# SysSec-KAIST/LTESniffer

Measured on AMD Instinct MI355X. Metric: subframes/s (20 MHz, 150 RNTIs), higher is better.
Workload: dtype f32+int16

## Files before the change

include/ltesniffer_amd.h:

```cpp
#ifndef LTESNIFFER_AMD_H
#define LTESNIFFER_AMD_H
#include <stddef.h>
#include <stdint.h>
#ifdef __cplusplus
extern "C" {
#endif

#define LSN_SUCCESS 0
#define LSN_ERROR (-1)
#define LSN_ERROR_INVALID_INPUTS (-2)
#define LSN_ERROR_NO_DEVICE (-3)

typedef struct lsn_phy lsn_phy_t;
typedef struct lsn_worker lsn_worker_t;

typedef struct {
  uint32_t nof_prb;
  uint32_t nof_ports;
  uint32_t id;
  uint32_t cp;
  uint32_t phich_length;
  uint32_t phich_resources;
  uint32_t frame_type;
} lsn_cell_t;
// ... 198 lines not shown
  float offset_freq_hz;
  uint32_t start_tti;
  uint32_t update_meta_period;
  uint64_t max_subframes;
  uint64_t subframes_done;
  int status;
} lsn_file_cell_t;
int lsn_file_process_cells(const char* path, const lsn_file_cfg_t* cfg , double sample_rate_hz,
                           lsn_file_cell_t* cells, uint32_t n_cells);
typedef struct {
  int64_t in_lo, in_hi;
  uint32_t blk_used, nof_active;
  uint64_t first_subframe[LSN_FILE_MAX_CELLS];
  uint32_t nof_subframes[LSN_FILE_MAX_CELLS];
  uint32_t taps[LSN_FILE_MAX_CELLS];
} lsn_file_cells_span_t;
int lsn_file_cells_span(const lsn_file_cfg_t* cfg, double sample_rate_hz, const lsn_file_cell_t* cells, uint32_t n_cells, uint64_t in_end ,
                        uint32_t block, uint32_t blk_subframes, lsn_file_cells_span_t* out);
int lsn_resample_cells(int device, const void* in, int in_on_device, uint64_t n_in, const lsn_resample_cfg_t* cfgs, uint32_t n_cells, float* const* outs,
                       int out_on_device, const uint64_t* n_out);

int lsn_resample_cells_ring(int device, const void* in, uint64_t n_in, uint64_t ring_samples, const lsn_resample_cfg_t* cfgs, uint32_t n_cells, float* const* outs,
                            const uint64_t* n_out);

typedef struct lsn_stream lsn_stream_t;
typedef struct {
  uint32_t struct_size;
  int      device;
  double   sample_rate_hz;
  uint32_t nof_antennas;
  uint32_t sample_format;
  float    sample_scale;
  uint32_t block_subframes;
  uint64_t ring_samples;
} lsn_stream_cfg_t;
typedef struct {
  uint64_t samples_pushed;
  uint64_t ring_samples;
  int64_t  oldest_needed;
  uint32_t block_subframes, nof_cells;
  int      failed;
  int      status[LSN_FILE_MAX_CELLS];
  uint64_t subframes_submitted[LSN_FILE_MAX_CELLS];
} lsn_stream_status_t;
typedef struct {
  uint64_t ring_samples, block_input;
// ... 282 lines not shown
```

ltesniffer_amd/__init__.py:

```python
import ctypes as C
import os
import struct
import subprocess

import numpy as np


_HERE = os.path.dirname(os.path.abspath(__file__))
LIB_PATH = os.environ.get("LSN_LIB_PATH") or os.path.join(_HERE, "lib", "libltesniffer_amd.so")

LSN_SUCCESS, LSN_ERROR, LSN_ERROR_INVALID_INPUTS, LSN_ERROR_NO_DEVICE = 0, -1, -2, -3
TAP_GRID, TAP_CE, TAP_PDCCH_LLR, TAP_CHEST, TAP_CFI, TAP_CANDIDATES, TAP_CCE_POWER, TAP_ACCEPTED, TAP_RB_POWER = range(9)
TAP_PDSCH_JOBS, TAP_PDSCH_LLR16, TAP_RM_WORDS, TAP_CB_RESULT = 9, 10, 11, 12
KERNELS = ["k_ofdm", "k_chest", "k_chest_fin", "k_pcfich", "k_pdcch_llr", "k_cce_power", "k_viterbi", "k_pdsch_prep",
           "k_pdsch_demod", "k_turbo<64>", "k_rb_power", "k_turbo<128>", "k_rm"]

EXPORTS = ["lsn_phy_create", "lsn_phy_destroy", "lsn_phy_set_cell", "lsn_phy_get_avail", "lsn_phy_put_pending",
           "lsn_phy_join_pending", "lsn_phy_set_pdu_sink", "lsn_phy_get_stats", "lsn_phy_get_est_cfo",
           "lsn_phy_add_evergreen", "lsn_phy_add_forbidden", "lsn_phy_setup_default_rnti_intervals",
           "lsn_phy_nof_active_rnti", "lsn_phy_get_ue_config", "lsn_worker_buffers", "lsn_worker_buffer_len", "lsn_worker_prepare",
           "lsn_worker_sf_idx", "lsn_worker_sfn", "lsn_phy_process_device", "lsn_phy_process_host", "lsn_phy_process_host_int", "lsn_phy_tap",
           "lsn_phy_get_perf", "lsn_kernel_name", "lsn_version", "lsn_pcap_open", "lsn_pcap_open_mem",
           "lsn_pcap_set_wall_clock", "lsn_pcap_write", "lsn_pcap_sink", "lsn_pcap_mem", "lsn_pcap_nof_records",
           "lsn_pcap_reset", "lsn_pcap_close", "lsn_phy_set_pcap_writer", "lsn_phy_set_api_mode", "lsn_phy_tracked_ul_modulation", "lsn_phy_set_ul_config", "lsn_phy_get_ul_config", "lsn_sib2_decode", "lsn_phy_pusch_decode",
           "lsn_phy_tap_ul", "lsn_phy_set_prach_config", "lsn_phy_prach_detect", "lsn_phy_set_prach_sink", "lsn_prach_tti_opportunity", "lsn_phy_process_file", "lsn_phy_mib_decode", "lsn_phy_mib_decode_llr", "lsn_phy_submit_device", "lsn_phy_wait", "lsn_cell_search",
           "lsn_phy_set_shortcut_discovery", "lsn_phy_get_shortcut_discovery", "lsn_phy_set_histogram_threshold", "lsn_phy_print_stats",
           "lsn_phy_set_mcs_update_interval", "lsn_phy_update_mcs_database", "lsn_phy_nof_tracked_rnti", "lsn_worker_buffers_offset", "lsn_pcap_digest", "lsn_pcap_set_store", "lsn_pcap_set_digest_blocks", "lsn_pcap_block_digests", "lsn_phy_create_multi", "lsn_phy_nof_devices",
           "lsn_phy_set_cfo_correction", "lsn_phy_get_cfo_correction", "lsn_phy_set_candidate_pruning", "lsn_phy_set_stage_c_taps", "lsn_phy_prepare_file", "lsn_phy_get_meta_formats", "lsn_phy_nof_workers", "lsn_phy_worker",
           "lsn_phy_set_sampling", "lsn_phy_get_sampling", "lsn_symbol_sz", "lsn_sampling_freq_hz", "lsn_cell_search_rates",
           "lsn_resample", "lsn_resample_span", "lsn_phy_process_file_rate", "lsn_resample_cells", "lsn_file_cells_span", "lsn_file_process_cells",
           "lsn_clock_plan", "lsn_clock_fit", "lsn_clock_replica", "lsn_clock_track", "lsn_clock_estimate", "lsn_file_clock_estimate",
           "lsn_carrier_scan_plan", "lsn_carrier_scan_decide", "lsn_carrier_scan", "lsn_file_carrier_scan", "lsn_carrier_channel", "lsn_carrier_channel_span",
           "lsn_phy_set_channel_filter", "lsn_channel_filter_design", "lsn_channel_filter", "lsn_channel_filter_span", "lsn_cells_stopbands",
           "lsn_resample_cells_ring", "lsn_stream_open", "lsn_stream_push", "lsn_stream_flush", "lsn_stream_status", "lsn_stream_close", "lsn_stream_span",
           "lsn_stream_track", "lsn_stream_track_status", "lsn_stream_track_step", "lsn_pss_timing", "lsn_pss_timing_error"]

RATES_3GPP, RATES_SRSRAN = 0, 1


def symbol_sz(nof_prb, rates=RATES_3GPP):
    return int(lib().lsn_symbol_sz(int(nof_prb), int(rates)))


def sampling_freq_hz(nof_prb, rates=RATES_3GPP):
    return int(lib().lsn_sampling_freq_hz(int(nof_prb), int(rates)))


def turbo_nwin(K):
    p1 = p2 = 1
    for P in range(min(K // 32, 128), 0, -1):
        if K % P == 0:
            p2 = P
            break
    for P in range(min(K // 32, 64), 0, -1):
        if K % P == 0:
            p1 = P
            break
    return p2 if p2 >= 96 else p1
# ... 342 lines not shown
        L.lsn_phy_set_pcap_writer.argtypes = [C.c_void_p, C.c_void_p]
        L.lsn_phy_set_ul_config.argtypes = [C.c_void_p, C.POINTER(UlCfg)]
        L.lsn_phy_tracked_ul_modulation.argtypes = [C.c_void_p, C.c_uint16]
        L.lsn_phy_set_api_mode.argtypes = [C.c_void_p, C.c_int, API_SINK, C.c_void_p, C.c_void_p]
        L.lsn_phy_get_ul_config.argtypes = [C.c_void_p, C.POINTER(UlCfg), C.POINTER(Sib2), C.POINTER(C.c_uint32)]
        L.lsn_sib2_decode.argtypes = [C.c_char_p, C.c_uint32, C.POINTER(Sib2)]
        L.lsn_phy_pusch_decode.argtypes = [C.c_void_p, C.c_void_p, C.c_int, C.c_uint32, C.c_uint32, C.c_void_p, C.c_uint32, C.c_void_p,
                                           C.c_void_p, C.c_size_t]
        L.lsn_phy_tap_ul.argtypes = [C.c_void_p, C.c_int, C.c_uint32, C.c_void_p, C.c_size_t]
        L.lsn_phy_tap_ul.restype = C.c_long
        L.lsn_phy_submit_device.argtypes = [C.c_void_p, C.c_void_p, C.c_uint32, C.c_uint32, C.c_uint32, C.c_void_p]
        L.lsn_phy_wait.argtypes = [C.c_void_p]
        L.lsn_phy_mib_decode.argtypes = [C.c_void_p, C.c_void_p, C.c_int, C.POINTER(Mib)]
        L.lsn_phy_mib_decode_llr.argtypes = [C.c_void_p, C.c_void_p, C.c_int, C.POINTER(Mib), C.c_void_p]
        L.lsn_phy_process_file.argtypes = [C.c_void_p, C.c_char_p, C.POINTER(FileCfg), C.c_uint32, C.c_uint64, C.c_uint32, C.POINTER(C.c_uint64)]
        L.lsn_phy_prepare_file.argtypes = [C.c_void_p, C.c_uint32]
        L.lsn_phy_process_file_rate.argtypes = [C.c_void_p, C.c_char_p, C.POINTER(FileCfg), C.POINTER(FileRate), C.c_uint32, C.c_uint64, C.c_uint32, C.POINTER(C.c_uint64)]
        L.lsn_resample.argtypes = [C.c_int, C.c_void_p, C.c_int, C.c_uint64, C.POINTER(ResampleCfg), C.c_void_p, C.c_int, C.c_uint64]
        L.lsn_resample_span.argtypes = [C.POINTER(ResampleCfg), C.c_uint64, C.c_uint64, C.POINTER(ResampleSpan)]
        L.lsn_resample_cells.argtypes = [C.c_int, C.c_void_p, C.c_int, C.c_uint64, C.POINTER(ResampleCfg), C.c_uint32, C.POINTER(C.c_void_p), C.c_int, C.POINTER(C.c_uint64)]
        L.lsn_file_cells_span.argtypes = [C.POINTER(FileCfg), C.c_double, C.POINTER(FileCell), C.c_uint32, C.c_uint64, C.c_uint32, C.c_uint32, C.POINTER(FileCellsSpan)]
        L.lsn_file_process_cells.argtypes = [C.c_char_p, C.POINTER(FileCfg), C.c_double, C.POINTER(FileCell), C.c_uint32]
        L.lsn_resample_cells_ring.argtypes = [C.c_int, C.c_void_p, C.c_uint64, C.c_uint64, C.POINTER(ResampleCfg), C.c_uint32, C.POINTER(C.c_void_p), C.POINTER(C.c_uint64)]
        L.lsn_stream_open.argtypes = [C.POINTER(StreamCfg), C.POINTER(FileCell), C.c_uint32, C.POINTER(C.c_void_p)]
        L.lsn_stream_push.argtypes = [C.c_void_p, C.c_void_p, C.c_uint64]
        L.lsn_stream_flush.argtypes = [C.c_void_p]
        L.lsn_stream_status.argtypes = [C.c_void_p, C.POINTER(StreamStatus)]
        L.lsn_stream_close.argtypes = [C.c_void_p]
        L.lsn_stream_span.argtypes = [C.POINTER(StreamCfg), C.POINTER(FileCell), C.c_uint32, C.c_uint64, C.POINTER(StreamSpan)]
        L.lsn_stream_track.argtypes = [C.c_void_p, C.POINTER(StreamTrackCfg)]
        L.lsn_stream_track_status.argtypes = [C.c_void_p, C.POINTER(StreamTrackStatus)]
        L.lsn_stream_track_step.argtypes = [C.POINTER(StreamTrackCfg), C.c_double, C.c_double, C.c_uint32, C.POINTER(StreamTrackState), C.c_double, C.c_int,
                                            C.POINTER(C.c_uint64), C.POINTER(C.c_uint64)]
        L.lsn_pss_timing.argtypes = [C.c_int, C.c_int, C.POINTER(PssTimingCell), C.c_uint32]
        L.lsn_pss_timing_error.argtypes = [C.c_void_p, C.c_uint32, C.POINTER(C.c_double), C.POINTER(C.c_double)]
        L.lsn_phy_set_prach_config.argtypes = [C.c_void_p, C.POINTER(PrachCfg)]
        L.lsn_phy_prach_detect.argtypes = [C.c_void_p, C.c_void_p, C.c_int, C.c_uint32, C.c_uint32, C.POINTER(PrachDet), C.c_uint32]
        L.lsn_phy_set_prach_sink.argtypes = [C.c_void_p, PRACH_SINK, C.c_void_p]
        L.lsn_phy_set_prach_sink.restype = None
        L.lsn_prach_tti_opportunity.argtypes = [C.c_uint32, C.c_uint32]
        L.lsn_phy_set_shortcut_discovery.argtypes = [C.c_void_p, C.c_int]
        L.lsn_phy_get_shortcut_discovery.argtypes = [C.c_void_p]
        L.lsn_phy_set_histogram_threshold.argtypes = [C.c_void_p, C.c_uint32]
        L.lsn_phy_print_stats.argtypes = [C.c_void_p, C.c_void_p]
        L.lsn_phy_set_mcs_update_interval.argtypes = [C.c_void_p, C.c_uint32]
        L.lsn_phy_update_mcs_database.argtypes = [C.c_void_p]
# ... 546 lines not shown
    n_in, nant = iq.shape[0], iq.shape[1]
    n = len(cells)
    cfgs = (ResampleCfg * max(n, 1))()
    counts = (C.c_uint64 * max(n, 1))()
    outs = []
    for i, c in enumerate(cells):
        cfgs[i] = _resample_cfg(nant, rate_in, c["rate_out"], c.get("first_sample", 0), c.get("first_frac", 0.0), in_base, c.get("out_first", 0), c.get("passband_hz", 0.0),
                                sample_format, sample_scale, c.get("center_offset_hz", 0.0))
        k = c.get("n_out", n_out)
        if k is None:
            sp = ResampleSpan()
            _check(lib().lsn_resample_span(C.byref(cfgs[i]), 0, int(in_base) + n_in, C.byref(sp)), "lsn_resample_span")
            k = int(sp.max_out)
        counts[i] = int(k)
        outs.append(np.zeros((nant, int(k)), dtype=np.complex64))
    ptrs = (C.c_void_p * max(n, 1))(*[o.ctypes.data for o in outs])
    rc = lib().lsn_resample_cells_ring(device, iq.ctypes.data, n_in, int(ring_samples), cfgs, n, ptrs, counts)
    if rc == LSN_ERROR_INVALID_INPUTS:
        raise ValueError("resample_cells_ring: refused")
    _check(rc, "lsn_resample_cells_ring")
    return outs


def channel_filter_design(rate_in, passband_hz, stopband_hz):
    import numpy as np
    d = ChannelFilterDesign(C.sizeof(ChannelFilterDesign), 0, 0, 0, 0.0)
    taps = np.zeros(2 * 512 + 1, dtype=np.float32)
    rc = lib().lsn_channel_filter_design(float(rate_in), float(passband_hz), float(stopband_hz), C.byref(d), taps.ctypes.data, taps.size)
    if rc == LSN_ERROR_INVALID_INPUTS:
        raise ValueError("channel filter: refused")
    _check(rc, "lsn_channel_filter_design")
    return dict(L=int(d.half_len), fc=float(d.cutoff), taps=taps[:d.nof_taps].copy())


def _channel_filter_cfg(nof_antennas, rate_in, passband_hz, stopband_hz, center_offset_hz, in_base, out_first, sample_format, sample_scale):
    return ChannelFilterCfg(C.sizeof(ChannelFilterCfg), int(nof_antennas), int(sample_format), float(sample_scale), float(rate_in), float(passband_hz), float(stopband_hz),
                            float(center_offset_hz), int(in_base), int(out_first))


def channel_filter_span(n_out, in_end, rate_in, passband_hz, stopband_hz, out_first=0, center_offset_hz=0.0):
    cfg = _channel_filter_cfg(1, rate_in, passband_hz, stopband_hz, center_offset_hz, 0, out_first, FILE_CF32, 0.0)
    sp = ResampleSpan()
    rc = lib().lsn_channel_filter_span(C.byref(cfg), int(n_out), int(in_end), C.byref(sp))
    if rc == LSN_ERROR_INVALID_INPUTS:
        raise ValueError("channel filter: refused")
    _check(rc, "lsn_channel_filter_span")
# ... 392 lines not shown
```

ltesniffer_amd/csrc/host/lsn_capi.cc:

```cpp
#include "lsn_engine.h"
#include "lsn_cells.h"
#include "lsn_chanfilt_launch.h"
#include "lsn_stream_ring.h"
#include <chrono>
#include <condition_variable>
#include <deque>
#include <mutex>
#include <thread>
#include <time.h>

struct lsn_worker {
  lsn_phy* phy = nullptr;
  float* buf[LSN_MAX_RX] = {nullptr, nullptr};
  float* buf_offset[2] = {nullptr, nullptr};
  uint32_t buf_len = 0;
  uint32_t index = 0;
  uint32_t sf_idx = 0, sfn = 0;
  int update_meta = 0;
  lsn_dl_sf_cfg_t sf_cfg{};
};

struct lsn_phy {
  std::unique_ptr<lsn::Engine> engine;
  std::vector<std::unique_ptr<lsn::Engine>> more;
// ... 767 lines not shown
      raw = d_in;
    }
    cf32* dst = (cf32*)out;
    const size_t out_bytes = (size_t)n_out * nant * sizeof(cf32);
    if (!out_on_device) {
      HIP_CHECK(hipMalloc(&d_out, out_bytes));
      dst = (cf32*)d_out;
    }
    LsnChanFirCell k;
    k.taps = d_taps; k.L = f.L; k.w = f.tune; k.nco = d_nco; k.out = dst; k.out_first = (int64_t)cfg->out_first; k.n_out = n_out;
    lsn_launch_chan_fir(raw, fmt, sfm.scale, need_lo, len, nant, &k, 1, st);
    if (!out_on_device) HIP_CHECK(hipMemcpyAsync(out, d_out, out_bytes, hipMemcpyDeviceToHost, st));
    HIP_CHECK(hipStreamSynchronize(st));
  } catch (const std::exception& ex) {
    fprintf(stderr, "ltesniffer_amd: channel_filter: %s\n", ex.what());
    rc = LSN_ERROR;
  }
  if (st) (void)hipStreamDestroy(st);
  if (d_in) (void)hipFree(d_in);
  if (d_taps) (void)hipFree(d_taps);
  if (d_out) (void)hipFree(d_out);
  return rc;
}
int lsn_phy_prepare_file(lsn_phy_t* phy, uint32_t nof_antennas)
{
  if (!phy) return LSN_ERROR_INVALID_INPUTS;
  return phy->engine->reserveFileBuffers(nof_antennas);
}
int lsn_phy_set_ul_config(lsn_phy_t* phy, const lsn_ul_cfg_t* cfg)
{
  if (!phy || !cfg) return LSN_ERROR_INVALID_INPUTS;
  return phy->engine->setUlConfig(*cfg);
}
static void sib2_to_c(const lsn::Sib2Config& c, lsn_sib2_t* o)
{
  o->n_sb = c.n_sb; o->hopping_mode = c.hopping_mode; o->pusch_hop_offset = c.pusch_hop_offset; o->enable_64qam = c.enable_64qam;
  o->group_hopping_enabled = c.group_hopping_enabled; o->group_assignment_pusch = c.group_assignment_pusch;
  o->sequence_hopping_enabled = c.sequence_hopping_enabled; o->cyclic_shift = c.cyclic_shift;
  o->root_seq_idx = c.root_seq_idx; o->prach_config_idx = c.prach_config_idx; o->high_speed_flag = c.high_speed_flag;
  o->zero_corr_zone = c.zero_corr_zone; o->prach_freq_offset = c.prach_freq_offset;
}
int lsn_phy_get_ul_config(lsn_phy_t* phy, lsn_ul_cfg_t* ul, lsn_sib2_t* sib2, uint32_t* from_sib2)
{
  if (!phy) return LSN_ERROR_INVALID_INPUTS;
  lsn::Sib2Config s;
  if (!phy->engine->getUlConfig(ul, nullptr, &s)) return 0;
// ... 105 lines not shown
```

ltesniffer_amd/csrc/kernels/lsn_rm.h:

```cpp
#pragma once
#include <stdint.h>
#ifndef LSN_HD
#ifdef __HIPCC__
#define LSN_HD __host__ __device__ __forceinline__
#else
#define LSN_HD static inline
#endif
#endif

struct LsnRmGeom {
  int K, D, R, KP, ND, F, Ncb, nn, nn0, k0, cum_k0;
  int pre01[33];
  int pre2[33];
  uint8_t cnt01[32];
  uint8_t first2[32];
};

LSN_HD int lsn_perm_tc_f(int c) { return ((c & 1) << 4) | ((c & 2) << 2) | (c & 4) | ((c & 8) >> 2) | ((c & 16) >> 4); }

LSN_HD int lsn_rm_nb01_cr(const LsnRmGeom& g, int col, int row)
{
  if (col >= 32) return g.pre01[32];
  const int c = g.cnt01[col];
  return g.pre01[col] + (row < c ? row : c);
// ... 79 lines not shown
LSN_HD int lsn_rm_col_of(int y)
{
#ifdef __HIP_DEVICE_COMPILE__
  return (int)(__builtin_bitreverse32((uint32_t)y) >> 27);
#else
  return lsn_perm_tc_f(y & 31);
#endif
}
LSN_HD void lsn_rm_rank01_fast(LsnRmCol e, int nn, int y, int* r0, int* r1)
{
  const int row = y >> 5, cnt = e.a & 255, m = row < cnt ? row : cnt;
  int a = (e.a >> 8) + row - m;
  int b = (e.b >> 8) + 2 * row - m - (row > 0 ? (e.b & 1) : 0);
  *r0 = a < 0 ? a + nn : a;
  *r1 = b < 0 ? b + nn : b;
}
LSN_HD int lsn_rm_rank2_fast(LsnRmCol e, int nn, int z)
{
  const int row = z >> 5, cnt = e.a & 255, m = row < cnt ? row : cnt;
  const int b = (e.b >> 8) + 2 * row - m - (row > 0 ? (e.b & 1) : 0) + (row < cnt ? 0 : 1);
  return b < 0 ? b + nn : b;
}

LSN_HD int lsn_turbo_nwin(int K)
{
  int p1 = 1, p2 = 1;
  for (int P = (K / 32 < 128 ? K / 32 : 128); P >= 1; P--)
    if (K % P == 0) { p2 = P; break; }
  for (int P = (K / 32 < 64 ? K / 32 : 64); P >= 1; P--)
    if (K % P == 0) { p1 = P; break; }
  return p2 >= 96 ? p2 : p1;
}
#define LSN_TURBO_ONE_WAVE_KMAX 3072
LSN_HD int lsn_turbo_il_words(int K) { const int P = lsn_turbo_nwin(K), W = K / P; return ((W + 1) / 2) * P; }
LSN_HD bool lsn_turbo_two_wave_class(int K) { return lsn_turbo_nwin(K) > 64 || K > LSN_TURBO_ONE_WAVE_KMAX; }
```

ltesniffer_amd/csrc/kernels/lsn_rows.h:

```cpp
#pragma once
#include <stdint.h>
#ifndef LSN_HD
#ifdef __HIPCC__
#define LSN_HD __host__ __device__ __forceinline__
#else
#define LSN_HD static inline
#endif
#endif

#define LSN_ROWS_PER_ITEM 16u
#define LSN_ROWS_DIV_SHIFT 20

struct LsnRowGeom {
  uint32_t n[2];
  uint32_t div_m[2];
  uint32_t rows0;
  uint32_t rows;
};

LSN_HD uint32_t lsn_rows_ordinal(const uint32_t mask[4], uint32_t prb)
{
  uint32_t n = 0;
  for (uint32_t w = 0; w < 4; w++) {
    const uint32_t lo = 32u * w;
// ... 10 lines not shown
    g.n[s] = lsn_rows_ordinal(prb_mask[s], nof_prb);
    g.div_m[s] = g.n[s] ? (1u << LSN_ROWS_DIV_SHIFT) / g.n[s] + 1u : 0u;
  }
  g.rows0 = (nslot - l0) * g.n[0];
  g.rows = g.rows0 + nslot * g.n[1];
  return g;
}

LSN_HD uint32_t lsn_rows_items(const LsnRowGeom& g) { return (g.rows + LSN_ROWS_PER_ITEM - 1u) / LSN_ROWS_PER_ITEM; }

LSN_HD void lsn_rows_locate(const LsnRowGeom& g, uint32_t l0, uint32_t nslot, uint32_t row, uint32_t* l, uint32_t* slot, uint32_t* ord)
{
  const uint32_t s = row >= g.rows0 ? 1u : 0u;
  const uint32_t r = s ? row - g.rows0 : row, n = s ? g.n[1] : g.n[0], m = s ? g.div_m[1] : g.div_m[0];
  const uint32_t q = (r * m) >> LSN_ROWS_DIV_SHIFT;
  *slot = s;
  *l = (s ? nslot : l0) + q;
  *ord = r - q * n;
}

LSN_HD uint32_t lsn_rows_sym_off(uint32_t nof_prb) { return 14u * nof_prb; }
LSN_HD uint32_t lsn_rows_list_off(uint32_t nof_prb) { return 14u * nof_prb + 16u; }
LSN_HD uint32_t lsn_rows_prefix_len(uint32_t nof_prb) { return 15u * nof_prb + 16u; }
```

ltesniffer_amd/csrc/kernels/stage_c.hip:

```cpp
#include "lsn_dsp.h"
#include <algorithm>
#include "lsn_rm.h"
#include <type_traits>

#define SQRT1_2F 0.70710678118654752440f
#define SQRT2F 1.41421356237309504880f
#define LLR_Q 180.0f

__global__ __launch_bounds__(64) void k_pdsch_prep_up(LsnCellDev c, const LsnGrantDev* __restrict__ jobs_h, LsnGrantDev* __restrict__ jobs_d, uint32_t njobs,
                                                      LsnCopySegs sg, uint16_t* __restrict__ prefix)
{
  const int lane = threadIdx.x, nprb = (int)c.nof_prb;
  if (blockIdx.x >= njobs) {
    const uint32_t w = blockIdx.x - njobs, nw = gridDim.x - njobs;
    for (uint32_t q = 0; q < sg.n; q++) {
      const uint32_t words = sg.words[q];
      const bool al = ((((uintptr_t)sg.src[q]) | ((uintptr_t)sg.dst[q])) & 15u) == 0;
      const uint32_t n16 = al ? words / 4 : 0;
      const uint4* a4 = (const uint4*)sg.src[q];
      uint4* b4 = (uint4*)sg.dst[q];
      for (uint32_t i = w * 64u + (uint32_t)lane; i < n16; i += nw * 64u) b4[i] = a4[i];
      const uint32_t* a = (const uint32_t*)sg.src[q];
      uint32_t* b = (uint32_t*)sg.dst[q];
      for (uint32_t i = n16 * 4 + w * 64u + (uint32_t)lane; i < words; i += nw * 64u) b[i] = a[i];
    }
    return;
  }
  __shared__ LsnGrantDev gs;
  constexpr int NW = (int)(sizeof(LsnGrantDev) / 4);
  static_assert(NW <= 64 && sizeof(LsnGrantDev) % 4 == 0, "one word per lane");
  if (lane < NW) {
    const uint32_t v = ((const uint32_t*)(jobs_h + blockIdx.x))[lane];
    ((uint32_t*)&gs)[lane] = v;
    ((uint32_t*)(jobs_d + blockIdx.x))[lane] = v;
  }
  __syncthreads();
  const LsnGrantDev& g = gs;
  uint16_t* pf = prefix + g.prefix_off;
  const int cls = g.sf_idx == 0 ? 0 : (g.sf_idx == 5 ? 1 : 2);
  uint32_t before = 0;
  for (int l = 0; l < 14; l++) {
    uint32_t run = 0;
    for (int base = 0; base < nprb; base += 64) {
      const int prb = base + lane;
      uint32_t v = 0;
      if (prb < nprb && l >= (int)g.l0 && ((g.prb_mask[l >= (int)c.nslot ? 1 : 0][prb >> 5] >> (prb & 31)) & 1u)) v = (uint32_t)__popc((unsigned)c.validmask[(cls * 14 + l) * nprb + prb]);
      uint32_t inc = v;
#pragma unroll
      for (int off = 1; off < 64; off <<= 1) {
        const uint32_t t = __shfl_up(inc, off);
        if (lane >= off) inc += t;
      }
      if (prb < nprb) pf[l * nprb + prb] = (uint16_t)(run + inc - v);
      run += __shfl(inc, 63);
    }
    if (lane == 0) pf[lsn_rows_sym_off((uint32_t)nprb) + l] = (uint16_t)before;
    before += run;
  }
  if (lane == 0) pf[lsn_rows_sym_off((uint32_t)nprb) + 14] = (uint16_t)before;
  uint8_t* pl = (uint8_t*)(pf + lsn_rows_list_off((uint32_t)nprb));
  for (int s = 0; s < 2; s++)
    for (int prb = lane; prb < nprb; prb += 64)
      if ((g.prb_mask[s][prb >> 5] >> (prb & 31)) & 1u) pl[s * nprb + (int)lsn_rows_ordinal(g.prb_mask[s], (uint32_t)prb)] = (uint8_t)prb;
}
void lsn_launch_pdsch_prep_up(const LsnCellDev& c, const LsnGrantDev* jobs_host, LsnGrantDev* jobs_dev, uint32_t njobs, const LsnCopySegs& sg, uint16_t* prefix, hipStream_t s)
{
  uint32_t total = 0;
  for (uint32_t q = 0; q < sg.n; q++) total += sg.words[q];
  const uint32_t ncopy = total ? std::max<uint32_t>(1u, std::min<uint32_t>((total / 4 + 63u) / 64u, 256u)) : 0u;
  LSN_LAUNCH(k_pdsch_prep_up, dim3(njobs + ncopy), dim3(64), 0, s, c, jobs_host, jobs_dev, njobs, sg, prefix);
}

__device__ __forceinline__ int lsn_cvt_sat(float r)
{
  int q;
  asm("v_cvt_i32_f32 %0, %1" : "=v"(q) : "v"(r));
  return q;
}
template <int QM>
__device__ __forceinline__ void emit_q(const LsnCellDev& c, cf32 x, float w, float inv_amp, uint32_t cinit, uint32_t idx, int16_t* __restrict__ out)
{
  float L[8];
  const float wq = w * LLR_Q;
  lsn_demod_llr(QM, x.r * inv_amp, x.i * inv_amp, L);
  const uint32_t n0 = idx * (uint32_t)QM;
  uint32_t x1w[2] = {0u, 0u}, m[8];
// ... 168 lines not shown
        float det = a * d - (br * br + bi * bi);
        cf32 x0, x1;
        x0.r = (d * z0r - (br * z1r - bi * z1i)) / det;
        x0.i = (d * z0i - (br * z1i + bi * z1r)) / det;
        x1.r = (a * z1r - (br * z0r + bi * z0i)) / det;
        x1.i = (a * z1i - (br * z0i - bi * z0r)) / det;
        float w0 = det / d * 4.0f / chan_ref, w1 = det / a * 4.0f / chan_ref;
        if (g.qm[0]) emit(c, (int)g.qm[0], x0, w0, inv_amp, g.cinit[0], idx, out0);
        if (g.qm[1]) emit(c, (int)g.qm[1], x1, w1, inv_amp, g.cinit[1], idx, out1);
      }
      break;
    }
  }
#undef GRID
#undef CE
}
void lsn_launch_pdsch_demod(const LsnCellDev& c, const LsnGrantDev* g, const uint32_t* items, uint32_t nitems, const uint16_t* prefix, const cf32* grid,
                            const cf32* ce, const LsnChest* ch, int16_t* llr, hipStream_t s)
{
  if (nitems) LSN_LAUNCH(k_pdsch_demod, dim3(nitems), dim3(192), 0, s, c, g, items, prefix, grid, ce, ch, llr);
}

#define RM_NT 256
template <bool STAGED>
__device__ __forceinline__ int rm_sum(const int16_t* __restrict__ e, const int16_t* es, int rank, int E, int nn)
{
  int acc = 0;
  for (int k = rank; k < E; k += nn) acc += STAGED ? (int)es[k] : (int)e[k];
  return acc > LSN_LLR_CLIP ? LSN_LLR_CLIP : (acc < -LSN_LLR_CLIP ? -LSN_LLR_CLIP : acc);
}
__global__ __launch_bounds__(RM_NT) void k_rm(const LsnCbDev* __restrict__ cbs, const int16_t* __restrict__ llr, uint32_t* __restrict__ spp_g, uint32_t seg)
{
  extern __shared__ __attribute__((aligned(16))) unsigned char rm_smem[];
  __shared__ LsnRmGeom geom;
  __shared__ LsnRmCol tab[32];
  int16_t* es = (int16_t*)rm_smem;
  const LsnCbDev cb = cbs[blockIdx.x];
  const int tid = threadIdx.x, K = (int)cb.K, F = (int)cb.F, E = (int)cb.E;
  const int P = cb.nwin ? (int)cb.nwin : lsn_turbo_nwin(K), W = K / P;
  const int ND = 32 * ((K + 4 + 31) >> 5) - (K + 4);
  const int16_t* e = llr + cb.e_off;
  const bool staged = (uint32_t)E <= seg;
  if (tid < 64) {
    int c01 = 0, f2 = 0, c2 = 0;
    if (tid < 32) lsn_rm_geom_col(ND, F, tid, &c01, &f2, &c2);
    int i01 = c01, i2 = c2;
#pragma unroll
    for (int off = 1; off < 32; off <<= 1) {
      const int t = __shfl_up(i01, off), u = __shfl_up(i2, off);
      if (tid >= off) { i01 += t; i2 += u; }
    }
    if (tid < 32) { geom.cnt01[tid] = (uint8_t)c01; geom.first2[tid] = (uint8_t)f2; geom.pre01[tid] = i01 - c01; geom.pre2[tid] = i2 - c2; }
    if (tid == 31) { geom.pre01[32] = i01; geom.pre2[32] = i2; }
    __builtin_amdgcn_fence(__ATOMIC_RELEASE, "wavefront"); __builtin_amdgcn_wave_barrier(); __builtin_amdgcn_fence(__ATOMIC_ACQUIRE, "wavefront");
    if (tid == 0) lsn_rm_geom_finish(geom, K, F, (int)cb.rv);
    __builtin_amdgcn_fence(__ATOMIC_RELEASE, "wavefront"); __builtin_amdgcn_wave_barrier(); __builtin_amdgcn_fence(__ATOMIC_ACQUIRE, "wavefront");
    if (tid < 32) tab[tid] = lsn_rm_fast_col(geom, tid);
  }
  if (staged) {
    const uintptr_t a0 = (uintptr_t)e & ~(uintptr_t)15;
    const int skew = (int)(((uintptr_t)e - a0) >> 1);
    const uint4* src = (const uint4*)a0;
    const int end = skew + E, vend = end >> 3;
    for (int v = tid; v <= vend; v += RM_NT) {
      uint4 d = make_uint4(0u, 0u, 0u, 0u);
      if (8 * v < end) d = src[v];
      if (v == vend) {
        const int q = end & 7;
        const uint32_t keep = (q & 1) ? 0x0000FFFFu : 0u;
        switch (q >> 1) { case 0: d.x &= keep; break; case 1: d.y &= keep; break; case 2: d.z &= keep; break; default: d.w &= keep; break; }
      }
      ((uint4*)es)[v] = d;
    }
    es += skew;
  }
  __syncthreads();
  const int nn = geom.nn;
  uint32_t* out = spp_g + cb.spp_off;
  const bool single = staged && E <= nn;
  auto streams = [&](int x, int& v0, int& v1, int& v2) {
    const int y = x + ND;
    int r0, r1;
    lsn_rm_rank01_fast(tab[lsn_rm_col_of(y)], nn, y, &r0, &r1);
    const int r2 = lsn_rm_rank2_fast(tab[lsn_rm_col_of(y - 1)], nn, y - 1);
    if (single) {
      v0 = (int)es[r0 < E ? r0 : E]; v1 = (int)es[r1 < E ? r1 : E]; v2 = (int)es[r2 < E ? r2 : E];
    } else if (staged) {
      v0 = rm_sum<true>(e, es, r0, E, nn); v1 = rm_sum<true>(e, es, r1, E, nn); v2 = rm_sum<true>(e, es, r2, E, nn);
    } else {
      v0 = rm_sum<false>(e, es, r0, E, nn); v1 = rm_sum<false>(e, es, r1, E, nn); v2 = rm_sum<false>(e, es, r2, E, nn);
    }
  };
  int tq = tid / P, tr = tid - tq * P;
  const int dq = RM_NT / P, dr = RM_NT - dq * P;
  for (int t = tid; t < K; t += RM_NT, tq += dq, tr += dr) {
    if (tr >= P) { tr -= P; tq++; }
    const int x = (int)__umul24((uint32_t)tr, (uint32_t)W) + tq;
    int v0, v1, v2;
    streams(x, v0, v1, v2);
    if (x < F) v0 = v1 = -LSN_LLR_CLIP;
    out[t] = ((uint32_t)v0 & 0x3FFu) | (((uint32_t)v1 & 0x3FFu) << 10) | (((uint32_t)v2 & 0x3FFu) << 20);
  }
  if (tid < 4) {
    int v0, v1, v2;
    streams(K + tid, v0, v1, v2);
    out[K + tid] = (uint32_t)v0; out[K + 4 + tid] = (uint32_t)v1; out[K + 8 + tid] = (uint32_t)v2;
  }
}
void lsn_launch_rm(const LsnCbDev* cb, const int16_t* llr, uint32_t* spp, uint32_t ncb, uint32_t emax, hipStream_t s)
{
  static std::atomic<uint64_t> attr_done{0};
  lsn_func_max_lds((const void*)k_rm, 65536, attr_done, "k_rm");
  const uint32_t cap = (65536 - 32) / 2;
  const uint32_t seg = emax < cap ? emax : cap;
  const size_t lds = (((size_t)seg + 16) * 2 + 15) & ~(size_t)15;
  if (ncb) LSN_LAUNCH(k_rm, dim3(ncb), dim3(RM_NT), lds, s, cb, llr, spp, seg);
}

__global__ __launch_bounds__(256) void k_harq_combine(const LsnCbDev* __restrict__ cbs, const uint32_t* __restrict__ keep, uint32_t* pool, uint32_t* scratch, uint32_t copy)
{
  const LsnCbDev cb = cbs[blockIdx.x];
  const uint32_t place = cb.reserved >> 30, off = cb.reserved & 0x3FFFFFFFu;
  const uint32_t* a = (place == 0u ? (const uint32_t*)pool : place == 1u ? (const uint32_t*)scratch : keep) + off;
  const int K = (int)cb.K;
  if (copy) {
    uint32_t* d = pool + cb.spp_off;
    for (int t = threadIdx.x; t < K + 12; t += 256) d[t] = a[t];
    return;
  }
// ... 231 lines not shown
```

Before: 285,400.

## Precompute rate-match walk tables and fuse PDSCH prefix scan with DPP

Rewrites the rate-dematching kernel so each thread derives its LLR byte offsets from per-column walk bases precomputed in LDS. This replaces per-element rank arithmetic, using med3 clamping and direct LDS address-space loads, and specialises the kernel on mode and filler presence. The PDSCH prefix kernel packs two symbols and the PRB-list ordinal into one word and scans them with DPP, which removes the separate PRB list pass and the shuffle-based scan. It also adds a standalone lsn_rm_blocks test entry point. The risk is correctness around the packed bit fields and the filler/head handling.

Result: no change. 289,300, median of 6 (+1.4%).

```diff
diff --git a/include/ltesniffer_amd.h b/include/ltesniffer_amd.h
--- a/include/ltesniffer_amd.h
+++ b/include/ltesniffer_amd.h
@@ -244,6 +244,11 @@
 
 int lsn_resample_cells_ring(int device, const void* in, uint64_t n_in, uint64_t ring_samples, const lsn_resample_cfg_t* cfgs, uint32_t n_cells, float* const* outs,
                             const uint64_t* n_out);
+
+typedef struct {
+  uint32_t K, F, E, rv, nwin, e_off, spp_off;
+} lsn_rm_block_t;
+int lsn_rm_blocks(int device, uint32_t n, const lsn_rm_block_t* blocks, const int16_t* e, uint64_t n_e, uint32_t* words, uint64_t n_words);
 
 typedef struct lsn_stream lsn_stream_t;
 typedef struct {
diff --git a/ltesniffer_amd/__init__.py b/ltesniffer_amd/__init__.py
--- a/ltesniffer_amd/__init__.py
+++ b/ltesniffer_amd/__init__.py
@@ -33,7 +33,7 @@
            "lsn_carrier_scan_plan", "lsn_carrier_scan_decide", "lsn_carrier_scan", "lsn_file_carrier_scan", "lsn_carrier_channel", "lsn_carrier_channel_span",
            "lsn_phy_set_channel_filter", "lsn_channel_filter_design", "lsn_channel_filter", "lsn_channel_filter_span", "lsn_cells_stopbands",
            "lsn_resample_cells_ring", "lsn_stream_open", "lsn_stream_push", "lsn_stream_flush", "lsn_stream_status", "lsn_stream_close", "lsn_stream_span",
-           "lsn_stream_track", "lsn_stream_track_status", "lsn_stream_track_step", "lsn_pss_timing", "lsn_pss_timing_error"]
+           "lsn_stream_track", "lsn_stream_track_status", "lsn_stream_track_step", "lsn_pss_timing", "lsn_pss_timing_error", "lsn_rm_blocks"]
 
 RATES_3GPP, RATES_SRSRAN = 0, 1
 
@@ -422,6 +422,7 @@
         L.lsn_file_cells_span.argtypes = [C.POINTER(FileCfg), C.c_double, C.POINTER(FileCell), C.c_uint32, C.c_uint64, C.c_uint32, C.c_uint32, C.POINTER(FileCellsSpan)]
         L.lsn_file_process_cells.argtypes = [C.c_char_p, C.POINTER(FileCfg), C.c_double, C.POINTER(FileCell), C.c_uint32]
         L.lsn_resample_cells_ring.argtypes = [C.c_int, C.c_void_p, C.c_uint64, C.c_uint64, C.POINTER(ResampleCfg), C.c_uint32, C.POINTER(C.c_void_p), C.POINTER(C.c_uint64)]
+        L.lsn_rm_blocks.argtypes = [C.c_int, C.c_uint32, C.POINTER(RmBlock), C.c_void_p, C.c_uint64, C.c_void_p, C.c_uint64]
         L.lsn_stream_open.argtypes = [C.POINTER(StreamCfg), C.POINTER(FileCell), C.c_uint32, C.POINTER(C.c_void_p)]
         L.lsn_stream_push.argtypes = [C.c_void_p, C.c_void_p, C.c_uint64]
         L.lsn_stream_flush.argtypes = [C.c_void_p]
@@ -1014,6 +1015,24 @@
     return outs
 
 
+class RmBlock(C.Structure):
+    _fields_ = [(n, C.c_uint32) for n in ("K", "F", "E", "rv", "nwin", "e_off", "spp_off")]
+
+
+def rm_blocks(blocks, e, n_words, device=0):
+    import numpy as np
+    e = np.ascontiguousarray(e, dtype=np.int16)
+    arr = (RmBlock * max(len(blocks), 1))()
+    for i, b in enumerate(blocks):
+        arr[i] = RmBlock(int(b["K"]), int(b["F"]), int(b["E"]), int(b["rv"]), int(b.get("nwin", 0)), int(b["e_off"]), int(b["spp_off"]))
+    words = np.zeros(int(n_words), dtype=np.uint32)
+    rc = lib().lsn_rm_blocks(device, len(blocks), arr, e.ctypes.data, e.size, words.ctypes.data, words.size)
+    if rc == LSN_ERROR_INVALID_INPUTS:
+        raise ValueError("rm_blocks: refused")
+    _check(rc, "lsn_rm_blocks")
+    return words
+
+
 def channel_filter_design(rate_in, passband_hz, stopband_hz):
     import numpy as np
     d = ChannelFilterDesign(C.sizeof(ChannelFilterDesign), 0, 0, 0, 0.0)
diff --git a/ltesniffer_amd/csrc/host/lsn_capi.cc b/ltesniffer_amd/csrc/host/lsn_capi.cc
--- a/ltesniffer_amd/csrc/host/lsn_capi.cc
+++ b/ltesniffer_amd/csrc/host/lsn_capi.cc
@@ -813,6 +813,49 @@
   if (d_out) (void)hipFree(d_out);
   return rc;
 }
+int lsn_rm_blocks(int device, uint32_t n, const lsn_rm_block_t* blocks, const int16_t* e, uint64_t n_e, uint32_t* words, uint64_t n_words)
+{
+  if (!n || n > 65535u || !blocks || !e || !words || n_e >= (1ull << 31) || n_words >= (1ull << 31)) return LSN_ERROR_INVALID_INPUTS;
+  std::vector<LsnCbDev> cbs(n);
+  uint32_t emax = 0;
+  for (uint32_t i = 0; i < n; i++) {
+    const lsn_rm_block_t& b = blocks[i];
+    uint32_t f1, f2;
+    if (!lsn::qpp_params((int)b.K, f1, f2) || b.F > 63u || b.F + 24u >= b.K || b.rv > 3u || !b.E || (uint64_t)b.e_off + b.E > n_e ||
+        (uint64_t)b.spp_off + b.K + 12u > n_words || (b.nwin && (b.nwin > 128u || b.K % b.nwin)))
+      return LSN_ERROR_INVALID_INPUTS;
+    LsnCbDev cb{};
+    cb.e_off = b.e_off; cb.E = b.E; cb.K = b.K; cb.F = b.F; cb.rv = b.rv; cb.spp_off = b.spp_off; cb.nwin = b.nwin; cb.dep = LSN_CB_NODEP;
+    cbs[i] = cb;
+    emax = std::max(emax, b.E);
+  }
+  const size_t e_bytes = ((size_t)n_e + 8) * sizeof(int16_t), w_bytes = (size_t)n_words * sizeof(uint32_t);
+  void *d_cb = nullptr, *d_e = nullptr, *d_w = nullptr;
+  hipStream_t st = nullptr;
+  int rc = LSN_SUCCESS;
+  try {
+    HIP_CHECK(hipSetDevice(device));
+    HIP_CHECK(hipStreamCreateWithFlags(&st, hipStreamNonBlocking));
+    HIP_CHECK(hipMalloc(&d_cb, (size_t)n * sizeof(LsnCbDev)));
+    HIP_CHECK(hipMalloc(&d_e, e_bytes));
+    HIP_CHECK(hipMalloc(&d_w, w_bytes));
+    HIP_CHECK(hipMemsetAsync(d_e, 0, e_bytes, st));
+    HIP_CHECK(hipMemcpyAsync(d_cb, cbs.data(), (size_t)n * sizeof(LsnCbDev), hipMemcpyHostToDevice, st));
+    HIP_CHECK(hipMemcpyAsync(d_e, e, (size_t)n_e * sizeof(int16_t), hipMemcpyHostToDevice, st));
+    HIP_CHECK(hipMemcpyAsync(d_w, words, w_bytes, hipMemcpyHostToDevice, st));
+    lsn_launch_rm((const LsnCbDev*)d_cb, (const int16_t*)d_e, (uint32_t*)d_w, n, emax, st);
+    HIP_CHECK(hipMemcpyAsync(words, d_w, w_bytes, hipMemcpyDeviceToHost, st));
+    HIP_CHECK(hipStreamSynchronize(st));
+  } catch (const std::exception& ex) {
+    fprintf(stderr, "ltesniffer_amd: rm_blocks: %s\n", ex.what());
+    rc = LSN_ERROR;
+  }
+  if (st) (void)hipStreamDestroy(st);
+  if (d_cb) (void)hipFree(d_cb);
+  if (d_e) (void)hipFree(d_e);
+  if (d_w) (void)hipFree(d_w);
+  return rc;
+}
 int lsn_phy_prepare_file(lsn_phy_t* phy, uint32_t nof_antennas)
 {
   if (!phy) return LSN_ERROR_INVALID_INPUTS;
diff --git a/ltesniffer_amd/csrc/kernels/lsn_rm.h b/ltesniffer_amd/csrc/kernels/lsn_rm.h
--- a/ltesniffer_amd/csrc/kernels/lsn_rm.h
+++ b/ltesniffer_amd/csrc/kernels/lsn_rm.h
@@ -125,6 +125,28 @@
   return b < 0 ? b + nn : b;
 }
 
+struct LsnRmWalk { int32_t a0, b1, b2; };
+LSN_HD LsnRmWalk lsn_rm_walk_col(const LsnRmGeom& g, int c)
+{
+  const LsnRmCol e = lsn_rm_fast_col(g, c);
+  const int cnt = e.a & 255, f2 = e.b & 1, last = g.R - 1;
+  int a0 = (e.a >> 8) - cnt, b1 = (e.b >> 8) - cnt - f2, b2 = b1 + 1;
+  if (a0 + last < 0) a0 += g.nn;
+  if (b1 + 2 * last < 0) b1 += g.nn;
+  if (b2 + 2 * last < 0) b2 += g.nn;
+  LsnRmWalk o;
+  o.a0 = 2 * a0; o.b1 = 2 * b1; o.b2 = 2 * b2;
+  return o;
+}
+LSN_HD bool lsn_rm_walk_ok(int x, int F) { return F == 0 || x > F; }
+LSN_HD void lsn_rm_walk01(int a0, int b1, int y, int* r0b, int* r1b)
+{
+  const int row = y >> 5;
+  *r0b = a0 + 2 * row;
+  *r1b = b1 + 4 * row;
+}
+LSN_HD int lsn_rm_walk2(int b2, int z) { return b2 + 4 * (z >> 5); }
+
 LSN_HD int lsn_turbo_nwin(int K)
 {
   int p1 = 1, p2 = 1;
diff --git a/ltesniffer_amd/csrc/kernels/lsn_rows.h b/ltesniffer_amd/csrc/kernels/lsn_rows.h
--- a/ltesniffer_amd/csrc/kernels/lsn_rows.h
+++ b/ltesniffer_amd/csrc/kernels/lsn_rows.h
@@ -56,3 +56,10 @@
 LSN_HD uint32_t lsn_rows_sym_off(uint32_t nof_prb) { return 14u * nof_prb; }
 LSN_HD uint32_t lsn_rows_list_off(uint32_t nof_prb) { return 14u * nof_prb + 16u; }
 LSN_HD uint32_t lsn_rows_prefix_len(uint32_t nof_prb) { return 15u * nof_prb + 16u; }
+
+#define LSN_ROWS_MAX_PRB 110u
+#define LSN_ROWS_SCAN_RE_BITS 11
+#define LSN_ROWS_SCAN_ORD_BITS 7
+static_assert(12u * LSN_ROWS_MAX_PRB < (1u << LSN_ROWS_SCAN_RE_BITS), "a symbol's RE prefix fits its field");
+static_assert(LSN_ROWS_MAX_PRB < (1u << LSN_ROWS_SCAN_ORD_BITS), "a slot's PRB ordinal fits its field");
+static_assert(2 * LSN_ROWS_SCAN_RE_BITS + LSN_ROWS_SCAN_ORD_BITS <= 32, "three fields in one word");
diff --git a/ltesniffer_amd/csrc/kernels/stage_c.hip b/ltesniffer_amd/csrc/kernels/stage_c.hip
--- a/ltesniffer_amd/csrc/kernels/stage_c.hip
+++ b/ltesniffer_amd/csrc/kernels/stage_c.hip
@@ -7,6 +7,16 @@
 #define SQRT2F 1.41421356237309504880f
 #define LLR_Q 180.0f
 
+__device__ __forceinline__ uint32_t lsn_wave_scan_incl(uint32_t v)
+{
+  v += (uint32_t)__builtin_amdgcn_update_dpp(0, (int)v, 0x111, 0xF, 0xF, false);
+  v += (uint32_t)__builtin_amdgcn_update_dpp(0, (int)v, 0x112, 0xF, 0xF, false);
+  v += (uint32_t)__builtin_amdgcn_update_dpp(0, (int)v, 0x114, 0xF, 0xF, false);
+  v += (uint32_t)__builtin_amdgcn_update_dpp(0, (int)v, 0x118, 0xF, 0xF, false);
+  v += (uint32_t)__builtin_amdgcn_update_dpp(0, (int)v, 0x142, 0xA, 0xF, false);
+  v += (uint32_t)__builtin_amdgcn_update_dpp(0, (int)v, 0x143, 0xC, 0xF, false);
+  return v;
+}
 __global__ __launch_bounds__(64) void k_pdsch_prep_up(LsnCellDev c, const LsnGrantDev* __restrict__ jobs_h, LsnGrantDev* __restrict__ jobs_d, uint32_t njobs,
                                                       LsnCopySegs sg, uint16_t* __restrict__ prefix)
 {
@@ -37,31 +47,43 @@
   __syncthreads();
   const LsnGrantDev& g = gs;
   uint16_t* pf = prefix + g.prefix_off;
+  uint8_t* pl = (uint8_t*)(pf + lsn_rows_list_off((uint32_t)nprb));
   const int cls = g.sf_idx == 0 ? 0 : (g.sf_idx == 5 ? 1 : 2);
+  constexpr uint32_t RE_MASK = (1u << LSN_ROWS_SCAN_RE_BITS) - 1u;
+  uint32_t alloc[2];
+#pragma unroll
+  for (int r = 0; r < 2; r++) {
+    const int prb = 64 * r + lane;
+    alloc[r] = prb < nprb ? (((g.prb_mask[0][prb >> 5] >> (prb & 31)) & 1u) | (((g.prb_mask[1][prb >> 5] >> (prb & 31)) & 1u) << 1)) : 0u;
+  }
   uint32_t before = 0;
-  for (int l = 0; l < 14; l++) {
+  for (int p = 0; p < 7; p++) {
+    const int la = 2 * p, lb = la + 1, sa = la >= (int)c.nslot ? 1 : 0, sb = lb >= (int)c.nslot ? 1 : 0;
+    const bool ona = la >= (int)g.l0, onb = lb >= (int)g.l0;
     uint32_t run = 0;
-    for (int base = 0; base < nprb; base += 64) {
-      const int prb = base + lane;
-      uint32_t v = 0;
-      if (prb < nprb && l >= (int)g.l0 && ((g.prb_mask[l >= (int)c.nslot ? 1 : 0][prb >> 5] >> (prb & 31)) & 1u)) v = (uint32_t)__popc((unsigned)c.validmask[(cls * 14 + l) * nprb + prb]);
-      uint32_t inc = v;
-#pragma unroll
-      for (int off = 1; off < 64; off <<= 1) {
-        const uint32_t t = __shfl_up(inc, off);
-        if (lane >= off) inc += t;
-      }
-      if (prb < nprb) pf[l * nprb + prb] = (uint16_t)(run + inc - v);
-      run += __shfl(inc, 63);
-    }
-    if (lane == 0) pf[lsn_rows_sym_off((uint32_t)nprb) + l] = (uint16_t)before;
-    before += run;
+#pragma unroll
+    for (int r = 0; r < 2; r++) {
+      if (64 * r >= nprb) break;
+      const int prb = 64 * r + lane;
+      uint32_t va = 0, vb = 0;
+      if (ona && ((alloc[r] >> sa) & 1u)) va = (uint32_t)__popc((unsigned)c.validmask[(cls * 14 + la) * nprb + prb]);
+      if (onb && ((alloc[r] >> sb) & 1u)) vb = (uint32_t)__popc((unsigned)c.validmask[(cls * 14 + lb) * nprb + prb]);
+      const uint32_t listed = p < 2 ? (alloc[r] >> p) & 1u : 0u;
+      const uint32_t v = va | (vb << LSN_ROWS_SCAN_RE_BITS) | (listed << (2 * LSN_ROWS_SCAN_RE_BITS));
+      const uint32_t inc = lsn_wave_scan_incl(v), ex = run + inc - v;
+      if (prb < nprb) {
+        pf[la * nprb + prb] = (uint16_t)(ex & RE_MASK);
+        pf[lb * nprb + prb] = (uint16_t)((ex >> LSN_ROWS_SCAN_RE_BITS) & RE_MASK);
+      }
+      if (listed) pl[p * nprb + (int)(ex >> (2 * LSN_ROWS_SCAN_RE_BITS))] = (uint8_t)prb;
+      run += (uint32_t)__builtin_amdgcn_readlane((int)inc, 63);
+    }
+    if (lane == 0) pf[lsn_rows_sym_off((uint32_t)nprb) + la] = (uint16_t)before;
+    before += run & RE_MASK;
+    if (lane == 0) pf[lsn_rows_sym_off((uint32_t)nprb) + lb] = (uint16_t)before;
+    before += (run >> LSN_ROWS_SCAN_RE_BITS) & RE_MASK;
   }
   if (lane == 0) pf[lsn_rows_sym_off((uint32_t)nprb) + 14] = (uint16_t)before;
-  uint8_t* pl = (uint8_t*)(pf + lsn_rows_list_off((uint32_t)nprb));
-  for (int s = 0; s < 2; s++)
-    for (int prb = lane; prb < nprb; prb += 64)
-      if ((g.prb_mask[s][prb >> 5] >> (prb & 31)) & 1u) pl[s * nprb + (int)lsn_rows_ordinal(g.prb_mask[s], (uint32_t)prb)] = (uint8_t)prb;
 }
 void lsn_launch_pdsch_prep_up(const LsnCellDev& c, const LsnGrantDev* jobs_host, LsnGrantDev* jobs_dev, uint32_t njobs, const LsnCopySegs& sg, uint16_t* prefix, hipStream_t s)
 {
@@ -276,25 +298,90 @@
 }
 
 #define RM_NT 256
-template <bool STAGED>
-__device__ __forceinline__ int rm_sum(const int16_t* __restrict__ e, const int16_t* es, int rank, int E, int nn)
-{
+enum { RM_SINGLE = 0, RM_STAGED = 1, RM_GLOBAL = 2 };
+typedef const __attribute__((address_space(3))) int16_t* RmLds;
+template <int MODE>
+__device__ __forceinline__ int rm_value(const unsigned char* eg, int rb, uint32_t lo, int endb, int stepb)
+{
+  if (MODE == RM_SINGLE) {
+    uint32_t o;
+    asm("v_med3_u32 %0, %1, %2, %3" : "=v"(o) : "v"(rb), "v"(lo), "s"(endb));
+    return (int)*(RmLds)(uintptr_t)o;
+  }
   int acc = 0;
-  for (int k = rank; k < E; k += nn) acc += STAGED ? (int)es[k] : (int)e[k];
+  for (int k = rb; k < endb; k += stepb) acc += MODE == RM_STAGED ? (int)*(RmLds)(uintptr_t)(uint32_t)k : (int)*(const int16_t*)(eg + k);
   return acc > LSN_LLR_CLIP ? LSN_LLR_CLIP : (acc < -LSN_LLR_CLIP ? -LSN_LLR_CLIP : acc);
+}
+struct RmCtx {
+  const unsigned char* eg;
+  const LsnRmCol* tab;
+  const LsnRmWalk* walk;
+  uint32_t* out;
+  uint32_t lo;
+  int K, F, P, W, ND, nn, e0, endb;
+};
+template <int MODE, bool FILL>
+__device__ __forceinline__ void rm_words(const RmCtx& c, int tid)
+{
+  const int stepb = 2 * c.nn;
+  int tq = tid / c.P, tr = tid - tq * c.P;
+  const int dq = RM_NT / c.P, dr = RM_NT - dq * c.P;
+  tq += c.ND;
+  for (int t = tid; t < c.K; t += RM_NT, tq += dq, tr += dr) {
+    if (tr >= c.P) { tr -= c.P; tq++; }
+    const int y = (int)__umul24((uint32_t)tr, (uint32_t)c.W) + tq, z = y - 1;
+    if (FILL && y <= c.F + c.ND) continue;
+    const LsnRmWalk& wy = c.walk[y & 31];
+    const int w2 = c.walk[z & 31].b2;
+    int r0, r1;
+    lsn_rm_walk01(wy.a0, wy.b1, y, &r0, &r1);
+    const int r2 = lsn_rm_walk2(w2, z);
+    const uint32_t v0 = (uint32_t)rm_value<MODE>(c.eg, r0, c.lo, c.endb, stepb), v1 = (uint32_t)rm_value<MODE>(c.eg, r1, c.lo, c.endb, stepb),
+                   v2 = (uint32_t)rm_value<MODE>(c.eg, r2, c.lo, c.endb, stepb);
+    uint32_t pk = v0 << 22;
+    pk = __builtin_amdgcn_alignbit(v1, pk, 10);
+    pk = __builtin_amdgcn_alignbit(v2, pk, 10);
+    c.out[t] = pk >> 2;
+  }
+  const bool term = tid < 4, head = FILL && tid <= c.F;
+  if (term || head) {
+#pragma unroll
+    for (int h = 0; h < 2; h++) {
+      if (h == 0 ? !term : !head) continue;
+      const int x = h == 0 ? c.K + tid : tid, y = x + c.ND;
+      int r0, r1;
+      lsn_rm_rank01_fast(c.tab[lsn_rm_col_of(y)], c.nn, y, &r0, &r1);
+      const int r2 = lsn_rm_rank2_fast(c.tab[lsn_rm_col_of(y - 1)], c.nn, y - 1);
+      if (h == 1 && x < c.F) r0 = r1 = c.endb;
+      else { r0 = c.e0 + 2 * r0; r1 = c.e0 + 2 * r1; }
+      int v0 = rm_value<MODE>(c.eg, r0, c.lo, c.endb, stepb), v1 = rm_value<MODE>(c.eg, r1, c.lo, c.endb, stepb);
+      const int v2 = rm_value<MODE>(c.eg, c.e0 + 2 * r2, c.lo, c.endb, stepb);
+      if (h == 0) {
+        c.out[x] = (uint32_t)v0; c.out[x + 4] = (uint32_t)v1; c.out[x + 8] = (uint32_t)v2;
+      } else {
+        if (x < c.F) v0 = v1 = -LSN_LLR_CLIP;
+        const int xq = x / c.W;
+        c.out[(x - xq * c.W) * c.P + xq] = ((uint32_t)v0 & 0x3FFu) | (((uint32_t)v1 & 0x3FFu) << 10) | (((uint32_t)v2 & 0x3FFu) << 20);
+      }
+    }
+  }
 }
 __global__ __launch_bounds__(RM_NT) void k_rm(const LsnCbDev* __restrict__ cbs, const int16_t* __restrict__ llr, uint32_t* __restrict__ spp_g, uint32_t seg)
 {
   extern __shared__ __attribute__((aligned(16))) unsigned char rm_smem[];
   __shared__ LsnRmGeom geom;
   __shared__ LsnRmCol tab[32];
-  int16_t* es = (int16_t*)rm_smem;
+  __shared__ LsnRmWalk walk[32];
   const LsnCbDev cb = cbs[blockIdx.x];
   const int tid = threadIdx.x, K = (int)cb.K, F = (int)cb.F, E = (int)cb.E;
   const int P = cb.nwin ? (int)cb.nwin : lsn_turbo_nwin(K), W = K / P;
   const int ND = 32 * ((K + 4 + 31) >> 5) - (K + 4);
   const int16_t* e = llr + cb.e_off;
   const bool staged = (uint32_t)E <= seg;
+  const uintptr_t a0 = (uintptr_t)e & ~(uintptr_t)15;
+  const int skew = staged ? (int)(((uintptr_t)e - a0) >> 1) : 0;
+  const uint32_t lo = (uint32_t)(uintptr_t)(const __attribute__((address_space(3))) unsigned char*)rm_smem;
+  const int e0 = staged ? (int)lo + 2 * skew : 0;
   if (tid < 64) {
     int c01 = 0, f2 = 0, c2 = 0;
     if (tid < 32) lsn_rm_geom_col(ND, F, tid, &c01, &f2, &c2);
@@ -309,11 +396,14 @@
     __builtin_amdgcn_fence(__ATOMIC_RELEASE, "wavefront"); __builtin_amdgcn_wave_barrier(); __builtin_amdgcn_fence(__ATOMIC_ACQUIRE, "wavefront");
     if (tid == 0) lsn_rm_geom_finish(geom, K, F, (int)cb.rv);
     __builtin_amdgcn_fence(__ATOMIC_RELEASE, "wavefront"); __builtin_amdgcn_wave_barrier(); __builtin_amdgcn_fence(__ATOMIC_ACQUIRE, "wavefront");
-    if (tid < 32) tab[tid] = lsn_rm_fast_col(geom, tid);
+    if (tid < 32) {
+      tab[tid] = lsn_rm_fast_col(geom, tid);
+      LsnRmWalk w = lsn_rm_walk_col(geom, lsn_perm_tc_f(tid));
+      w.a0 += e0; w.b1 += e0; w.b2 += e0;
+      walk[tid] = w;
+    }
   }
   if (staged) {
-    const uintptr_t a0 = (uintptr_t)e & ~(uintptr_t)15;
-    const int skew = (int)(((uintptr_t)e - a0) >> 1);
     const uint4* src = (const uint4*)a0;
     const int end = skew + E, vend = end >> 3;
     for (int v = tid; v <= vend; v += RM_NT) {
@@ -324,41 +414,19 @@
         const uint32_t keep = (q & 1) ? 0x0000FFFFu : 0u;
         switch (q >> 1) { case 0: d.x &= keep; break; case 1: d.y &= keep; break; case 2: d.z &= keep; break; default: d.w &= keep; break; }
       }
-      ((uint4*)es)[v] = d;
-    }
-    es += skew;
+      ((uint4*)rm_smem)[v] = d;
+    }
   }
   __syncthreads();
-  const int nn = geom.nn;
-  uint32_t* out = spp_g + cb.spp_off;
-  const bool single = staged && E <= nn;
-  auto streams = [&](int x, int& v0, int& v1, int& v2) {
-    const int y = x + ND;
-    int r0, r1;
-    lsn_rm_rank01_fast(tab[lsn_rm_col_of(y)], nn, y, &r0, &r1);
-    const int r2 = lsn_rm_rank2_fast(tab[lsn_rm_col_of(y - 1)], nn, y - 1);
-    if (single) {
-      v0 = (int)es[r0 < E ? r0 : E]; v1 = (int)es[r1 < E ? r1 : E]; v2 = (int)es[r2 < E ? r2 : E];
-    } else if (staged) {
-      v0 = rm_sum<true>(e, es, r0, E, nn); v1 = rm_sum<true>(e, es, r1, E, nn); v2 = rm_sum<true>(e, es, r2, E, nn);
-    } else {
-      v0 = rm_sum<false>(e, es, r0, E, nn); v1 = rm_sum<false>(e, es, r1, E, nn); v2 = rm_sum<false>(e, es, r2, E, nn);
-    }
-  };
-  int tq = tid / P, tr = tid - tq * P;
-  const int dq = RM_NT / P, dr = RM_NT - dq * P;
-  for (int t = tid; t < K; t += RM_NT, tq += dq, tr += dr) {
-    if (tr >= P) { tr -= P; tq++; }
-    const int x = (int)__umul24((uint32_t)tr, (uint32_t)W) + tq;
-    int v0, v1, v2;
-    streams(x, v0, v1, v2);
-    if (x < F) v0 = v1 = -LSN_LLR_CLIP;
-    out[t] = ((uint32_t)v0 & 0x3FFu) | (((uint32_t)v1 & 0x3FFu) << 10) | (((uint32_t)v2 & 0x3FFu) << 20);
-  }
-  if (tid < 4) {
-    int v0, v1, v2;
-    streams(K + tid, v0, v1, v2);
-    out[K + tid] = (uint32_t)v0; out[K + 4 + tid] = (uint32_t)v1; out[K + 8 + tid] = (uint32_t)v2;
+  RmCtx c;
+  c.eg = (const unsigned char*)e; c.tab = tab; c.walk = walk; c.out = spp_g + cb.spp_off;
+  c.K = K; c.F = F; c.P = P; c.W = W; c.ND = ND; c.nn = geom.nn; c.lo = lo; c.e0 = e0; c.endb = e0 + 2 * E;
+  if (staged && E <= c.nn) {
+    if (F == 0) rm_words<RM_SINGLE, false>(c, tid); else rm_words<RM_SINGLE, true>(c, tid);
+  } else if (staged) {
+    if (F == 0) rm_words<RM_STAGED, false>(c, tid); else rm_words<RM_STAGED, true>(c, tid);
+  } else {
+    if (F == 0) rm_words<RM_GLOBAL, false>(c, tid); else rm_words<RM_GLOBAL, true>(c, tid);
   }
 }
 void lsn_launch_rm(const LsnCbDev* cb, const int16_t* llr, uint32_t* spp, uint32_t ncb, uint32_t emax, hipStream_t s)
```
